# pgvector/pgvector

Measured on AMD Instinct MI355X. Metric: QPS @ recall@10 (IVFFlat, 1M x 1536d), higher is better.
Workload: dtype f32

## Files before the change

### pgvector_amd/csrc/kernels_mfma.hip

```cpp
#include "pgv_device.h"

#include <algorithm>
#include <cfloat>

namespace pgv {

namespace {

typedef float f32x16 __attribute__((ext_vector_type(16)));
typedef _Float16 f16x8 __attribute__((ext_vector_type(8)));
typedef unsigned int u32x4 __attribute__((ext_vector_type(4)));

constexpr int kSliceBytes = 128;
#ifndef PGV_ARGMIN_AUX
#define PGV_ARGMIN_AUX 0
#endif
constexpr int kCand = 4;
constexpr int kWide = 8;

template <typename T> struct MfmaCfg;
template <> struct MfmaCfg<float> {
    static constexpr int WM = 2, WN = 2, TM = 2, TN = 2;
};
template <> struct MfmaCfg<__half> {
// ... 449 lines not shown
__global__ __launch_bounds__(256) void argmin_merge_kernel(int64_t n, int nparts, int lg, const float *__restrict__ part_val,
                                                           const int32_t *__restrict__ part_idx,
                                                           const float *__restrict__ part_x2,
                                                           const float *__restrict__ part_drop, int32_t *__restrict__ out_idx,
                                                           float *__restrict__ out_val, const L2Lists l2) {
    constexpr int W = NC > 1 ? kWide : 1;
    const int G = 1 << lg;
    const int64_t t = (int64_t)blockIdx.x * blockDim.x + threadIdx.x;
    const int64_t r = t >> lg;
    const int p = (int)(t & (G - 1));
    const bool live = r < n && p < nparts;
    unsigned long long list[NC];
#pragma unroll
    for (int c = 0; c < NC; c++) {
        list[c] = ~0ull;
        if (live) {
            const size_t at = ((size_t)r * nparts + p) * NC + c;
            const float v = part_val[at];
            if (v < INFINITY) list[c] = ((unsigned long long)float_to_key(v) << 32) | (unsigned)part_idx[at];
        }
    }
    float sv[W];
    int sid[W];
#pragma unroll
    for (int c = 0; c < W; c++) {
        unsigned long long best = list[0];
        for (int m = 1; m < G; m <<= 1) {
            const unsigned long long o = __shfl_xor(best, m);
            best = o < best ? o : best;
        }
        if (best == ~0ull) {
            sv[c] = INFINITY;
            sid[c] = 0;
        } else {
            sv[c] = key_to_float((unsigned)(best >> 32));
            sid[c] = (int)(unsigned)(best & 0xffffffffu);
        }
        if (list[0] == best && best != ~0ull) {
#pragma unroll
            for (int j = 0; j + 1 < NC; j++) list[j] = list[j + 1];
            list[NC - 1] = ~0ull;
        }
    }
    if constexpr (NC > 1) {
        float dropped = live ? part_drop[(size_t)r * nparts + p] : INFINITY;
        if (list[0] != ~0ull) dropped = fminf(dropped, key_to_float((unsigned)(list[0] >> 32)));
        for (int m = 1; m < G; m <<= 1) dropped = fminf(dropped, __shfl_xor(dropped, m));
        if (r < n && p == 0) finish_l2(r, sv, sid, dropped, part_x2[r], out_idx, l2);
    } else {
        if (r < n && p == 0) finish_ip(r, sv[0], sid[0], out_idx, out_val);
    }
}

template <typename T>
__global__ __launch_bounds__(256) void center_norms_kernel(const char *__restrict__ centers, int k, int nvec,
                                                           float *__restrict__ bias, unsigned *__restrict__ cmax2) {
    const int c = blockIdx.x * 4 + (threadIdx.x >> 6);
    if (c >= k) return;
    const int lane = threadIdx.x & (kWave - 1);
    const char *row = centers + (size_t)c * nvec * sizeof(Raw16);
    float acc = 0.f;
    for (int v = lane; v < nvec; v += kWave) {
        const Raw16 x = load16(row + (size_t)v * sizeof(Raw16));
        acc = accum_slice<T, 1>(acc, x, x);
    }
    for (int m = 32; m > 0; m >>= 1) acc += __shfl_xor(acc, m);
    if (lane == 0) {
        bias[c] = acc;
        atomicMax(cmax2, __float_as_uint(acc));
    }
}

template <typename T>
__global__ __launch_bounds__(256) void recheck_kernel(const char *__restrict__ rows, const char *__restrict__ centers,
                                                      int k, int nvec, const L2Lists l2, int32_t *__restrict__ out_idx,
                                                      int *__restrict__ fb_count,
                                                      int32_t *__restrict__ fb_rows,
                                                      unsigned long long *__restrict__ packed) {
    const int64_t p = (int64_t)blockIdx.x * 4 + (threadIdx.x >> 6);
    if (p >= *l2.u_count) return;
    const int64_t r = l2.u_rows[p];
    const int lane = threadIdx.x & (kWave - 1);
    const size_t row_bytes = (size_t)nvec * sizeof(Raw16);
    const char *row = rows + (size_t)r * row_bytes;
    const float cm2 = __uint_as_float(*l2.cmax2), x2 = l2.u_x2[p];
    const float v0 = l2.u_val[p * kWide];
    int ncheck = 2;
    while (ncheck < kWide && !out_of_band(l2.u_val[p * kWide + ncheck], v0, x2, cm2, l2.gamma, l2.gamma_x)) ncheck++;
    float bv = INFINITY;
    int bid = 0x7fffffff;
    for (int c0 = 0; c0 < ncheck; c0 += kCand) {
        int id[kCand];
        const char *cp[kCand];
#pragma unroll
        for (int c = 0; c < kCand; c++) {
            id[c] = l2.u_cand[p * kWide + (c0 + c < ncheck ? c0 + c : c0)];
            cp[c] = centers + (size_t)id[c] * row_bytes;
        }
        float d[kCand] = {0.f, 0.f, 0.f, 0.f};
        for (int v = lane; v < nvec; v += kWave) {
            const Raw16 x = load16(row + (size_t)v * sizeof(Raw16));
#pragma unroll
            for (int c = 0; c < kCand; c++) d[c] = accum_slice<T, 0>(d[c], x, load16(cp[c] + (size_t)v * sizeof(Raw16)));
        }
        for (int m = 32; m > 0; m >>= 1) {
#pragma unroll
            for (int c = 0; c < kCand; c++) d[c] += __shfl_xor(d[c], m);
        }
#pragma unroll
        for (int c = 0; c < kCand; c++)
            if (c0 + c < ncheck && l2.u_val[p * kWide + c0 + c] < INFINITY &&
                (d[c] < bv || (d[c] == bv && d[c] < INFINITY && id[c] < bid))) {
                bv = d[c];
                bid = id[c];
            }
    }
    if (lane != 0) return;
    out_idx[r] = bid == 0x7fffffff ? 0 : bid;
    if (k > kWide) {
        const bool list_ok = ncheck < kWide;
        if (!(list_ok && out_of_band(l2.u_drop[p], v0, x2, cm2, l2.gamma, l2.gamma_x))) {
            packed[r] = ~0ull;
            fb_rows[atomicAdd(fb_count, 1)] = (int32_t)r;
        }
    }
}

__global__ __launch_bounds__(256) void redo_finish_kernel(const int *__restrict__ fb_count,
                                                          const int32_t *__restrict__ fb_rows,
                                                          const unsigned long long *__restrict__ packed,
                                                          int32_t *__restrict__ out_idx) {
    const int64_t p = (int64_t)blockIdx.x * 256 + threadIdx.x;
    if (p >= *fb_count) return;
    const int64_t r = fb_rows[p];
    const unsigned long long e = packed[r];
    out_idx[r] = e == ~0ull ? 0 : (int32_t)(unsigned)(e & 0xffffffffu);
}

template <typename T>
__global__ __launch_bounds__(256) void chosen_distance_kernel(const char *__restrict__ rows, int64_t n,
                                                              const char *__restrict__ centers, int nvec,
                                                              const int32_t *__restrict__ idx,
                                                              float *__restrict__ out_val) {
    const int64_t r = (int64_t)blockIdx.x * 4 + (threadIdx.x >> 6);
    if (r >= n) return;
    const int lane = threadIdx.x & (kWave - 1);
    const size_t row_bytes = (size_t)nvec * sizeof(Raw16);
    const char *row = rows + (size_t)r * row_bytes;
    const char *cp = centers + (size_t)idx[r] * row_bytes;
    float d0 = 0.f, d1 = 0.f;
    int v = lane;
    for (; v + kWave < nvec; v += 2 * kWave) {
        const Raw16 x0 = load16(row + (size_t)v * sizeof(Raw16)), x1 = load16(row + (size_t)(v + kWave) * sizeof(Raw16));
        const Raw16 c0 = load16(cp + (size_t)v * sizeof(Raw16)), c1 = load16(cp + (size_t)(v + kWave) * sizeof(Raw16));
        d0 = accum_slice<T, 0>(d0, x0, c0);
        d1 = accum_slice<T, 0>(d1, x1, c1);
    }
    if (v < nvec) d0 = accum_slice<T, 0>(d0, load16(row + (size_t)v * sizeof(Raw16)), load16(cp + (size_t)v * sizeof(Raw16)));
    float d = d0 + d1;
    for (int m = 32; m > 0; m >>= 1) d += __shfl_xor(d, m);
    if (lane == 0) out_val[r] = d < INFINITY ? d : FLT_MAX;
}

__global__ void add_count_kernel(const int *u_count, const int *fb_count, double *acc, double rows) {
    acc[0] += (double)*fb_count;
    acc[1] += rows;
    acc[2] += (double)*u_count;
}

template <typename T, int MODE>
int launch_mfma_t(pgv_ctx *ctx, const RowGeom &g, const void *rows, int64_t n, const void *centers, int k,
                  const float *bias, int32_t *out_idx, float *out_val, const L2Lists &l2 = L2Lists()) {
    using C = MfmaCfg<T>;
    constexpr int BM = C::WM * C::TM * 32, BN = C::WN * C::TN * 32;
    constexpr int threads = C::WM * C::WN * 64;
    constexpr int NC = MODE == 0 ? kCand : 1;
    const size_t lds = 2 * (size_t)(BM + BN) * kSliceBytes + sizeof(float) * BM;
    auto kern = mfma_argmin_kernel<T, MODE>;
    PGV_HIP(hipFuncSetAttribute(reinterpret_cast<const void *>(kern), hipFuncAttributeMaxDynamicSharedMemorySize,
                                (int)lds));
    const int64_t row_tiles = (n + BN - 1) / BN;
    static const int env_tiles = [] {
        const char *e = getenv("PGV_ARGMIN_PART_TILES");
        return e ? atoi(e) : -1;
    }();
    const int center_tiles = (k + BM - 1) / BM;
    const bool split = MODE != 0 || sizeof(T) == 2 || row_tiles < 2 * (int64_t)ctx->num_cus;
    const int auto_tiles = row_tiles < 2 * (int64_t)ctx->num_cus ? 1 : (sizeof(T) == 2 ? (MODE == 0 ? 4 : 2) : 1);
    int part_tiles = env_tiles < 0 ? (split ? auto_tiles : center_tiles) : (env_tiles == 0 ? center_tiles : env_tiles);
    int nparts = (center_tiles + part_tiles - 1) / part_tiles;
    if (nparts > 64) {
        part_tiles = (center_tiles + 63) / 64;
        nparts = (center_tiles + part_tiles - 1) / part_tiles;
    }
    float *part_val = nullptr, *part_x2 = nullptr, *part_drop = nullptr;
    int32_t *part_idx = nullptr;
    int64_t grid = row_tiles;
    const bool norms_pass = MODE == 0 && (nparts > 1 || sizeof(T) == 2);
    if (nparts > 1 || norms_pass) {
        const size_t pv = sizeof(float) * (size_t)n * nparts * NC;
        const size_t pd = sizeof(float) * (size_t)n * nparts;
        PGV_TRY(ctx->mf_d.ensure(2 * pv + pd + sizeof(float) * (size_t)n + 64));
        part_val = ctx->mf_d.as<float>();
        part_idx = reinterpret_cast<int32_t *>(ctx->mf_d.as<char>() + pv);
        part_drop = reinterpret_cast<float *>(ctx->mf_d.as<char>() + 2 * pv);
        part_x2 = reinterpret_cast<float *>(ctx->mf_d.as<char>() + 2 * pv + pd);
        if (nparts > 1) grid = 8 * ((row_tiles + 7) / 8) * nparts;
    }
    if (grid > 0x7fffffff) PGV_FAIL(PGV_ERR_ARG, "assignment: too many workgroups");
    if (norms_pass) {
        unsigned *max_bits = reinterpret_cast<unsigned *>(part_x2 + n);
        PGV_HIP(hipMemsetAsync(max_bits, 0, sizeof(unsigned), ctx->stream));
        PGV_TRY(launch_row_norms(ctx, sizeof(T) == 4 ? PGV_F32 : PGV_F16, g, rows, n, part_x2, max_bits));
    }
    hipLaunchKernelGGL(kern, dim3((unsigned)grid), dim3(threads), lds, ctx->stream, static_cast<const char *>(rows), n,
                       static_cast<const char *>(centers), k, g.nvec, bias, static_cast<const char *>(ctx->zeros.p),
                       out_idx, out_val, l2, nparts, part_tiles, part_val, part_idx, part_x2, part_drop);
    PGV_HIP(hipGetLastError());
    if (nparts > 1) {
        int lg = 0;
        while ((1 << lg) < nparts) lg++;
        const int64_t threads_total = n << lg;
        hipLaunchKernelGGL(argmin_merge_kernel<NC>, dim3((unsigned)((threads_total + 255) / 256)), dim3(256), 0, ctx->stream, n,
                           nparts, lg, part_val, part_idx, part_x2, part_drop, out_idx, out_val, l2);
        PGV_HIP(hipGetLastError());
    }
    return PGV_OK;
}

template <typename T>
int launch_mfma_mode(pgv_ctx *ctx, int mode, const RowGeom &g, const void *rows, int64_t n, const void *centers, int k,
                     int32_t *out_idx, float *out_val) {
    if (mode == 1) return launch_mfma_t<T, 1>(ctx, g, rows, n, centers, k, nullptr, out_idx, out_val);
    if (mode == 3) return launch_mfma_t<T, 3>(ctx, g, rows, n, centers, k, nullptr, out_idx, out_val);

    const pgv_dtype dtype = sizeof(T) == 4 ? PGV_F32 : PGV_F16;
    PGV_TRY(ctx->mf_a.ensure(sizeof(float) * (size_t)k + 64));
    PGV_TRY(ctx->mf_b.ensure((sizeof(int32_t) + sizeof(float)) * (size_t)n * kWide + 2 * sizeof(float) * (size_t)n));
    PGV_TRY(ctx->mf_c.ensure((2 * sizeof(int32_t) + sizeof(unsigned long long)) * (size_t)n + 16));
    float *bias = ctx->mf_a.as<float>();
    unsigned *cmax2 = reinterpret_cast<unsigned *>(bias + k);
    int *u_count = reinterpret_cast<int *>(cmax2 + 1);
    int *fb_count = u_count + 1;
    int32_t *u_cand = ctx->mf_b.as<int32_t>();
    float *u_val = reinterpret_cast<float *>(u_cand + (size_t)n * kWide);
    unsigned long long *packed = ctx->mf_c.as<unsigned long long>();
    int32_t *u_rows = reinterpret_cast<int32_t *>(packed + n);
    int32_t *fb_rows = u_rows + n;
    PGV_HIP(hipMemsetAsync(cmax2, 0, 3 * sizeof(int), ctx->stream));
    hipLaunchKernelGGL(center_norms_kernel<T>, dim3((k + 3) / 4), dim3(256), 0, ctx->stream,
                       static_cast<const char *>(centers), k, g.nvec, bias, cmax2);
    L2Lists l2;
    l2.cmax2 = cmax2;
    const ExpansionBound eb = argmin_bound(ctx, g.ld);
    l2.gamma = eb.gamma;
    l2.gamma_x = eb.gamma_exact;
    l2.u_count = u_count;
    l2.u_rows = u_rows;
    l2.u_cand = u_cand;
    l2.u_val = u_val;
    l2.u_drop = u_val + (size_t)n * kWide;
    l2.u_x2 = l2.u_drop + n;
    PGV_TRY((launch_mfma_t<T, 0>(ctx, g, rows, n, centers, k, bias, out_idx, nullptr, l2)));
    hipLaunchKernelGGL(recheck_kernel<T>, dim3((unsigned)((n + 3) / 4)), dim3(256), 0, ctx->stream,
                       static_cast<const char *>(rows), static_cast<const char *>(centers), k, g.nvec, l2, out_idx, fb_count,
                       fb_rows, packed);
    PGV_HIP(hipGetLastError());
    if (k > kWide) {
        PGV_TRY(launch_argmin_listed(ctx, 0, dtype, g, rows, n, centers, k, fb_rows, fb_count, packed));
        hipLaunchKernelGGL(redo_finish_kernel, dim3((unsigned)((n + 255) / 256)), dim3(256), 0, ctx->stream, fb_count,
                           fb_rows, packed, out_idx);
        PGV_HIP(hipGetLastError());
    }
    if (out_val) {
        hipLaunchKernelGGL(chosen_distance_kernel<T>, dim3((unsigned)((n + 3) / 4)), dim3(256), 0, ctx->stream,
                           static_cast<const char *>(rows), n, static_cast<const char *>(centers), g.nvec, out_idx,
                           out_val);
        PGV_HIP(hipGetLastError());
    }
    if (ctx->profiling && ctx->stats_dev.p) {
        hipLaunchKernelGGL(add_count_kernel, dim3(1), dim3(1), 0, ctx->stream, u_count, fb_count,
                           ctx->stats_dev.as<double>() + 2, (double)n);
        PGV_HIP(hipGetLastError());
    }
    return PGV_OK;
}

constexpr int kScanQueries = 32;

constexpr int kScanWaves = 4;

template <typename T, int METRIC, int NW, bool NT, int NQ, int NS = 2, bool SH = false>
__global__ __launch_bounds__(NW * 64) __attribute__((amdgpu_waves_per_eu(NS == 3 ? 2 : 3, NS == 3 ? 2 : 3))) void mfma_scan_kernel(
    const char *__restrict__ rows, const char *__restrict__ queries, const ScanTask *__restrict__ tasks,
    const int *__restrict__ ntasks_ptr, int *__restrict__ task_counter, const ScanPair *__restrict__ pairs,
    const float *__restrict__ row_norms, int nvec, const char *__restrict__ zeros16, float *__restrict__ out,
    const float *__restrict__ qscale) {
    static_assert(!SH || (METRIC == 0 && sizeof(T) == 2), "the shadow scan: fp16 rows, L2");
    constexpr int ROWS = 32 * NW;
    constexpr int NGROUPS = (NQ + ROWS) / 8;
    constexpr int NDMA = (NGROUPS + NW - 1) / NW;
    constexpr int STAGE = (NQ + ROWS) * kSliceBytes;
    static_assert(NS == 2 || (NS == 3 && NQ == 32 && NGROUPS % NW == 0), "three stages: the 32-query form only");
    __shared__ __attribute__((aligned(16))) char smem[NS * STAGE];
    __shared__ int64_t pair_rel[NQ];
    __shared__ float2 pair_ts[SH ? NQ : 1];
    __shared__ int lds_task;
    auto value = [&](float acc, float rn) -> float {
        if constexpr (SH)
            return acc;
        else
            return METRIC == 0 ? fmaf(-2.f, acc, rn) : -acc;
    };
    auto shadow_values = [&](auto &acc, int n, float rn, auto slot) {
#pragma unroll
        for (int r = 0; r < n; r++) {
            const float2 ts = pair_ts[slot(r)];
            acc[r] = fmaf(-ts.y, acc[r], rn + ts.x);
        }
    };

    const int lane = threadIdx.x & (kWave - 1);
    const int wave = __builtin_amdgcn_readfirstlane(threadIdx.x >> 6);
    const int l31 = lane & 31, half = lane >> 5;
    const unsigned sw = (unsigned)(l31 >> 1) & 7u;
    const size_t row_bytes = (size_t)nvec * sizeof(Raw16);
    const int nslices = (nvec + 7) / 8;
    const int ntasks = *ntasks_ptr;
    const unsigned lds0 = (unsigned)(size_t)(__attribute__((address_space(3))) char *)smem;
    const int drow = lane >> 3, dpos = lane & 7;

    if (threadIdx.x == 0) lds_task = atomicAdd(task_counter, 1);
    __syncthreads();
    for (;;) {
        const int t = lds_task;
        if (t >= ntasks) {
            if (threadIdx.x == 0 && atomicAdd(task_counter + 1, 1) == (int)gridDim.x - 1) {
                task_counter[0] = 0;
                task_counter[1] = 0;
            }
            return;
        }
        int next = 0;
        if (threadIdx.x == 0) next = atomicAdd(task_counter, 1);
        const ScanTask task = tasks[t];
        const int np = task.npairs;
        if ((int)threadIdx.x < NQ) {
            const ScanPair pr = pairs[task.pair0 + ((int)threadIdx.x < np ? (int)threadIdx.x : np - 1)];
            pair_rel[threadIdx.x] = pr.out_rel + task.row0;
            if constexpr (SH) {
                pair_ts[threadIdx.x] = make_float2(__int_as_float(pr.pad), qscale[pr.query]);
            }
        }
        const char *src[NDMA];
#pragma unroll
        for (int j = 0; j < NDMA; j++) {
            const int crow = (wave + NW * j) * 8 + drow;
            if (crow < NQ) {
                const ScanPair pr = pairs[task.pair0 + (crow < np ? crow : np - 1)];
                src[j] = queries + (size_t)pr.query * row_bytes;
            } else {
                const int r = crow - NQ;
                src[j] = rows + ((size_t)task.row0 + (size_t)(r < task.nrows ? r : task.nrows - 1)) * row_bytes;
            }
        }
        const bool narrow = np <= 16;
        const bool upper = NQ > 32 && np > 32;
        const bool past_caches = NT && task.pad == 0;
        auto issue_stage = [&](int sl, int buf) {
#pragma unroll
            for (int j = 0; j < NDMA; j++) {
                const int g8 = wave + NW * j;
                if (NGROUPS % NW != 0 && g8 >= NGROUPS) break;
                if (narrow && g8 >= 2 && g8 < NQ / 8) continue;
                if (NQ > 32 && !upper && g8 >= 4 && g8 < NQ / 8) continue;
                const int v = dpos ^ ((4 * (g8 & 1) + (drow >> 1)) & 7);
                const int vi = sl * 8 + v;
                const char *p = vi < nvec ? src[j] + (size_t)vi * sizeof(Raw16) : zeros16;
                char *dst = smem + (size_t)buf * STAGE + (size_t)g8 * 8 * kSliceBytes;
                if (NT && past_caches && g8 >= NQ / 8)
                    __builtin_amdgcn_global_load_lds((const __attribute__((address_space(1))) void *)p,
                                                     (__attribute__((address_space(3))) void *)dst, 16, 0, 2);
                else
                    __builtin_amdgcn_global_load_lds((const __attribute__((address_space(1))) void *)p,
                                                     (__attribute__((address_space(3))) void *)dst, 16, 0, 0);
            }
        };
        const int j32 = wave * 32 + l31;
        if constexpr (NQ > 32) {
          if (!narrow && upper) {
            f32x16 accl, accu, suml, sumu;
#pragma unroll
            for (int r = 0; r < 16; r++) {
                accl[r] = 0.f;
                accu[r] = 0.f;
                suml[r] = 0.f;
                sumu[r] = 0.f;
            }
            const int quarter = (nslices + 3) >> 2;
            int in_quarter = 0;
            const unsigned a_lane = (unsigned)l31 * kSliceBytes;
            const unsigned b_lane = (unsigned)(NQ + wave * 32 + l31) * kSliceBytes;
            issue_stage(0, 0);
            for (int sl = 0; sl < nslices; sl++) {
                __builtin_amdgcn_s_waitcnt(0x0070);
                __builtin_amdgcn_s_barrier();
                if (sl + 1 < nslices) issue_stage(sl + 1, (sl + 1) & 1);
                const unsigned sbase = lds0 + (unsigned)(sl & 1) * STAGE;
                if (upper) {
#pragma unroll
                    for (int c = 0; c < 4; c++) {
                        const unsigned x = (((unsigned)(2 * c + half)) ^ sw) << 4;
                        u32x4 a, au, b;
                        asm volatile("ds_read_b128 %0, %3\n\tds_read_b128 %1, %3 offset:4096\n\tds_read_b128 %2, %4\n\t"
                                     "s_waitcnt lgkmcnt(0)"
                                     : "=&v"(a), "=&v"(au), "=&v"(b)
                                     : "v"(sbase + a_lane + x), "v"(sbase + b_lane + x)
                                     : "memory");
                        Mma<T>::run(accl, a, b);
                        Mma<T>::run(accu, au, b);
                    }
                } else {
#pragma unroll
                    for (int c = 0; c < 4; c++) {
                        const unsigned x = (((unsigned)(2 * c + half)) ^ sw) << 4;
                        u32x4 a, b;
                        asm volatile("ds_read_b128 %0, %2\n\tds_read_b128 %1, %3\n\ts_waitcnt lgkmcnt(0)"
                                     : "=&v"(a), "=&v"(b)
                                     : "v"(sbase + a_lane + x), "v"(sbase + b_lane + x)
                                     : "memory");
                        Mma<T>::run(accl, a, b);
                    }
                }
                if (++in_quarter == quarter) {
                    in_quarter = 0;
                    suml += accl;
                    sumu += accu;
#pragma unroll
                    for (int r = 0; r < 16; r++) {
                        accl[r] = 0.f;
                        accu[r] = 0.f;
                    }
                }
            }
            suml += accl;
            sumu += accu;
            const int j32w = wave * 32 + l31;
            if (j32w < task.nrows) {
                const float rn = METRIC == 0 ? row_norms[task.row0 + j32w] : 0.f;
                if constexpr (SH) {
                    shadow_values(suml, 16, rn, [&](int r) { return (r & 3) + 8 * (r >> 2) + 4 * half; });
                    if (upper) shadow_values(sumu, 16, rn, [&](int r) { return 32 + (r & 3) + 8 * (r >> 2) + 4 * half; });
                }
                {
                    int64_t rel[16];
#pragma unroll
                    for (int r = 0; r < 16; r++) rel[r] = pair_rel[(r & 3) + 8 * (r >> 2) + 4 * half];
#pragma unroll
                    for (int r = 0; r < 16; r++) out[rel[r] + j32w] = value(suml[r], rn);
                }
                if (upper) {
                    int64_t rel[16];
#pragma unroll
                    for (int r = 0; r < 16; r++) rel[r] = pair_rel[32 + (r & 3) + 8 * (r >> 2) + 4 * half];
#pragma unroll
                    for (int r = 0; r < 16; r++) out[rel[r] + j32w] = value(sumu[r], rn);
                }
            }
          }
        }
        if (!narrow && !upper) {
            f32x16 acc4[4];
#pragma unroll
            for (int e = 0; e < 4; e++)
#pragma unroll
                for (int r = 0; r < 16; r++) acc4[e][r] = 0.f;
            const unsigned a_lane = (unsigned)l31 * kSliceBytes;
            const unsigned b_lane = (unsigned)(NQ + wave * 32 + l31) * kSliceBytes;
            issue_stage(0, 0);
            if (NS == 3 && nslices > 1) issue_stage(1, 1);
            int buf = 0;
            for (int sl = 0; sl < nslices; sl++) {
                if (NS == 3 && sl > 0 && sl + 1 < nslices)
                    __builtin_amdgcn_s_waitcnt(0x0075);
                else
                    __builtin_amdgcn_s_waitcnt(0x0070);
                __builtin_amdgcn_s_barrier();
                if (NS == 3) {
                    if (sl + 2 < nslices) issue_stage(sl + 2, buf == 0 ? 2 : buf - 1);
                } else {
                    if (sl + 1 < nslices) issue_stage(sl + 1, (sl + 1) & 1);
                }
                const unsigned sbase = lds0 + (unsigned)(NS == 3 ? buf : (sl & 1)) * STAGE;
                if (NS == 3) buf = buf == 2 ? 0 : buf + 1;
                if (NS == 3) {
                    u32x4 pa[2], pb[2];
                    const unsigned x0 = (((unsigned)half) ^ sw) << 4;
                    asm volatile("ds_read_b128 %0, %2\n\tds_read_b128 %1, %3"
                                 : "=&v"(pa[0]), "=&v"(pb[0])
                                 : "v"(sbase + a_lane + x0), "v"(sbase + b_lane + x0)
                                 : "memory");
#pragma unroll
                    for (int c = 0; c < 4; c++) {
                        if (c + 1 < 4) {
                            const unsigned x = (((unsigned)(2 * (c + 1) + half)) ^ sw) << 4;
                            asm volatile("ds_read_b128 %0, %2\n\tds_read_b128 %1, %3"
                                         : "=&v"(pa[(c + 1) & 1]), "=&v"(pb[(c + 1) & 1])
                                         : "v"(sbase + a_lane + x), "v"(sbase + b_lane + x)
                                         : "memory");
                            asm volatile("s_waitcnt lgkmcnt(2)" : "+v"(pa[c & 1]), "+v"(pb[c & 1])::"memory");
                        } else {
                            asm volatile("s_waitcnt lgkmcnt(0)" : "+v"(pa[c & 1]), "+v"(pb[c & 1])::"memory");
                        }
                        __builtin_amdgcn_sched_barrier(0);
                        Mma4<T>::run(acc4, pa[c & 1], pb[c & 1], c);
                        __builtin_amdgcn_sched_barrier(0);
                    }
                } else {
#pragma unroll
                    for (int c = 0; c < 4; c++) {
                        const unsigned x = (((unsigned)(2 * c + half)) ^ sw) << 4;
                        u32x4 a, b;
                        asm volatile("ds_read_b128 %0, %2\n\tds_read_b128 %1, %3\n\ts_waitcnt lgkmcnt(0)"
                                     : "=&v"(a), "=&v"(b)
                                     : "v"(sbase + a_lane + x), "v"(sbase + b_lane + x)
                                     : "memory");
                        Mma4<T>::run(acc4, a, b, c);
                    }
                }
            }
            f32x16 acc = (acc4[0] + acc4[1]) + (acc4[2] + acc4[3]);
            if constexpr (SH)
                shadow_values(acc, 16, j32 < task.nrows ? row_norms[task.row0 + j32] : 0.f,
                              [&](int r) { return (r & 3) + 8 * (r >> 2) + 4 * half; });
            int64_t rel[16];
#pragma unroll
            for (int r = 0; r < 16; r++) rel[r] = pair_rel[(r & 3) + 8 * (r >> 2) + 4 * half];
            if (j32 < task.nrows) {
                const float rn = METRIC == 0 ? row_norms[task.row0 + j32] : 0.f;
#pragma unroll
                for (int r = 0; r < 16; r++)
                    out[rel[r] + j32] = value(acc[r], rn);
            }
        }
        if (narrow) {
            const int l15 = lane & 15, kg = lane >> 4;
            const unsigned sw15 = (unsigned)(l15 >> 1) & 7u;
            f32x4 c04[4], c14[4];
#pragma unroll
            for (int e = 0; e < 4; e++) {
                c04[e] = f32x4{0.f, 0.f, 0.f, 0.f};
                c14[e] = f32x4{0.f, 0.f, 0.f, 0.f};
            }
            const unsigned a_lane = (unsigned)l15 * kSliceBytes;
            const unsigned b_lane = (unsigned)(NQ + wave * 32 + l15) * kSliceBytes;
            issue_stage(0, 0);
            for (int sl = 0; sl < nslices; sl++) {
                __builtin_amdgcn_s_waitcnt(0x0070);
                __builtin_amdgcn_s_barrier();
                if (sl + 1 < nslices) issue_stage(sl + 1, (sl + 1) & 1);
                const unsigned sbase = lds0 + (unsigned)(sl & 1) * STAGE;
#pragma unroll
                for (int c = 0; c < 2; c++) {
                    const unsigned x = (((unsigned)(kg + 4 * c)) ^ sw15) << 4;
                    u32x4 a, b0, b1;
                    asm volatile("ds_read_b128 %0, %3\n\tds_read_b128 %1, %4\n\tds_read_b128 %2, %4 offset:2048\n\t"
                                 "s_waitcnt lgkmcnt(0)"
                                 : "=&v"(a), "=&v"(b0), "=&v"(b1)
                                 : "v"(sbase + a_lane + x), "v"(sbase + b_lane + x)
                                 : "memory");
                    if (sl & 1)
                        Mma16x4<T>::run(c04, c14, a, b0, b1, c + 2);
                    else
                        Mma16x4<T>::run(c04, c14, a, b0, b1, c);
                }
            }
            f32x4 c0 = (c04[0] + c04[1]) + (c04[2] + c04[3]), c1 = (c14[0] + c14[1]) + (c14[2] + c14[3]);
            int64_t rel[4];
#pragma unroll
            for (int r = 0; r < 4; r++) rel[r] = pair_rel[4 * kg + r];
            const int ja = wave * 32 + l15, jb = ja + 16;
            const float rna = (METRIC == 0 && ja < task.nrows) ? row_norms[task.row0 + ja] : 0.f;
            const float rnb = (METRIC == 0 && jb < task.nrows) ? row_norms[task.row0 + jb] : 0.f;
            if constexpr (SH) {
                shadow_values(c0, 4, rna, [&](int r) { return 4 * kg + r; });
                shadow_values(c1, 4, rnb, [&](int r) { return 4 * kg + r; });
            }
            if (ja < task.nrows) {
#pragma unroll
                for (int r = 0; r < 4; r++) out[rel[r] + ja] = value(c0[r], rna);
            }
            if (jb < task.nrows) {
#pragma unroll
                for (int r = 0; r < 4; r++) out[rel[r] + jb] = value(c1[r], rnb);
            }
        }
        __builtin_amdgcn_s_waitcnt(0xc07f);
        __builtin_amdgcn_s_barrier();
        if (threadIdx.x == 0) lds_task = next;
        __syncthreads();
    }
}

template <typename T>
__global__ __launch_bounds__(256) void row_norms_kernel(const char *__restrict__ rows, int64_t n, int nvec,
                                                        float *__restrict__ out, unsigned *__restrict__ max_bits) {
    const int64_t r = (int64_t)blockIdx.x * 4 + (threadIdx.x >> 6);
    if (r >= n) return;
    const int lane = threadIdx.x & (kWave - 1);
    const char *row = rows + (size_t)r * nvec * sizeof(Raw16);
    float acc = 0.f;
    for (int v = lane; v < nvec; v += kWave) {
        const Raw16 x = load16(row + (size_t)v * sizeof(Raw16));
        acc = accum_slice<T, 1>(acc, x, x);
    }
    for (int m = 32; m > 0; m >>= 1) acc += __shfl_xor(acc, m);
    if (lane == 0) {
        out[r] = acc;
        if (max_bits && __float_as_uint(acc) > __hip_atomic_load(max_bits, __ATOMIC_RELAXED, __HIP_MEMORY_SCOPE_AGENT))
            atomicMax(max_bits, __float_as_uint(acc));
    }
}

}

bool mfma_argmin_supported(int mode, int64_t n, int k) { return (mode == 0 || mode == 1 || mode == 3) && k >= 64 && n >= 256; }

int launch_argmin_mfma(pgv_ctx *ctx, int mode, pgv_dtype dtype, const RowGeom &g, const void *rows, int64_t n,
                       const void *centers, int k, int32_t *out_idx, float *out_val) {
    if (n <= 0) return PGV_OK;
    if (!ctx->zeros.p) {
        PGV_TRY(ctx->zeros.ensure(256));
        PGV_HIP(hipMemsetAsync(ctx->zeros.p, 0, 256, ctx->stream));
    }
    if (dtype == PGV_F32) return launch_mfma_mode<float>(ctx, mode, g, rows, n, centers, k, out_idx, out_val);
    return launch_mfma_mode<__half>(ctx, mode, g, rows, n, centers, k, out_idx, out_val);
}

}

namespace pgv {

int mfma_scan_rows_per_task() { return 32 * kScanWaves; }
int mfma_scan_queries_per_task() { return kScanQueries; }
int shadow_chain_length(const RowGeom &g16) {
    const int nslices = (g16.nvec + 7) / 8;
    const int a = 16 * nslices, b = 32 * ((nslices + 1) / 2), c = 64 * ((nslices + 3) / 4);
    return std::max(a, std::max(b, c));
}
int scan_chain_length(const RowGeom &g, pgv_dtype dtype, bool wide) {
    const int nslices = (g.nvec + 7) / 8, quarter = (nslices + 3) / 4;
    if (dtype == PGV_F32) return std::max(g.ld / 4, wide ? 32 * quarter : 0);
    return std::max(16 * nslices, std::max(32 * ((nslices + 1) / 2), wide ? 64 * quarter : 0));
}
int mfma_scan_queries_per_task_wide() { return 2 * kScanQueries; }

int launch_row_norms(pgv_ctx *ctx, pgv_dtype dtype, const RowGeom &g, const void *rows, int64_t n, float *out,
                     unsigned *max_bits) {
    if (n <= 0) return PGV_OK;
    const dim3 grid((unsigned)((n + 3) / 4));
    if (dtype == PGV_F32)
        hipLaunchKernelGGL(row_norms_kernel<float>, grid, dim3(256), 0, ctx->stream, static_cast<const char *>(rows), n,
                           g.nvec, out, max_bits);
    else
        hipLaunchKernelGGL(row_norms_kernel<__half>, grid, dim3(256), 0, ctx->stream, static_cast<const char *>(rows), n,
                           g.nvec, out, max_bits);
    PGV_HIP(hipGetLastError());
    return PGV_OK;
}

int launch_mfma_scan(pgv_ctx *ctx, pgv_metric metric, pgv_dtype dtype, const RowGeom &g, const void *rows,
                     const void *queries, const ScanTask *tasks, const int *ntasks_dev, int ntasks_bound,
                     const ScanPair *pairs, const float *row_norms, const float *query_norms, float *out,
                     bool stream_rows, int queries_per_task, const float *shadow_scale) {
    if (ntasks_bound <= 0) return PGV_OK;
    if (queries_per_task != 32 && queries_per_task != 64) PGV_FAIL(PGV_ERR_ARG, "mfma scan: %d queries per task", queries_per_task);
    if (metric != PGV_L2SQ && metric != PGV_NEG_IP) PGV_FAIL(PGV_ERR_ARG, "mfma scan: L2 / inner product only");
    if (!ctx->zeros.p) {
        PGV_TRY(ctx->zeros.ensure(256));
        PGV_HIP(hipMemsetAsync(ctx->zeros.p, 0, 256, ctx->stream));
    }
    PGV_TRY(ctx->counters.ensure(256));
    if (!ctx->counters_clean) {
        PGV_HIP(hipMemsetAsync(ctx->counters.p, 0, 256, ctx->stream));
        ctx->counters_clean = true;
    }
    int *counter = ctx->counters.as<int>() + 8;
    int grid = ctx->num_cus * 3;
    if (grid > ntasks_bound) grid = ntasks_bound;
    static const int deep_env = [] {
        const char *e = getenv("PGV_SCAN_DEEP");
        return e ? atoi(e) : -1;
    }();
    const bool deep = queries_per_task == 32 && deep_env != 0 && ntasks_bound <= 2 * ctx->num_cus;
#define PGV_MSCAN_QS(T, M, NT, Q, S, SH)                                                                                  \
    hipLaunchKernelGGL((mfma_scan_kernel<T, M, kScanWaves, NT, Q, S, SH>), dim3(grid), dim3(kScanWaves * 64), 0,          \
                       ctx->stream, static_cast<const char *>(rows), static_cast<const char *>(queries), tasks, ntasks_dev, \
                       counter, pairs, row_norms, g.nvec, static_cast<const char *>(ctx->zeros.p), out, shadow_scale)
#define PGV_MSCAN_Q(T, M, NT, Q, S) PGV_MSCAN_QS(T, M, NT, Q, S, false)
#define PGV_MSCAN_NT(T, M, NT)                   \
    do {                                         \
        if (queries_per_task == 64)              \
            PGV_MSCAN_Q(T, M, NT, 64, 2);         \
        else if (deep)                           \
            PGV_MSCAN_Q(T, M, NT, 32, 3);         \
        else                                     \
            PGV_MSCAN_Q(T, M, NT, 32, 2);         \
    } while (0)
#define PGV_MSCAN(T, M)              \
    do {                             \
        if (stream_rows)             \
            PGV_MSCAN_NT(T, M, true); \
        else                         \
            PGV_MSCAN_NT(T, M, false); \
    } while (0)
    if (shadow_scale) {
        if (metric != PGV_L2SQ || dtype != PGV_F16) PGV_FAIL(PGV_ERR_ARG, "mfma scan: the shadow form is fp16 L2 only");
#define PGV_MSCAN_SH(NT)                                   \
    do {                                                   \
        if (queries_per_task == 64)                        \
            PGV_MSCAN_QS(__half, 0, NT, 64, 2, true);       \
        else if (deep)                                     \
            PGV_MSCAN_QS(__half, 0, NT, 32, 3, true);       \
        else                                               \
            PGV_MSCAN_QS(__half, 0, NT, 32, 2, true);       \
    } while (0)
        if (stream_rows)
            PGV_MSCAN_SH(true);
        else
            PGV_MSCAN_SH(false);
#undef PGV_MSCAN_SH
    } else if (dtype == PGV_F32) {
        if (metric == PGV_L2SQ)
            PGV_MSCAN(float, 0);
        else
            PGV_MSCAN(float, 1);
    } else {
        if (metric == PGV_L2SQ)
            PGV_MSCAN(__half, 0);
        else
            PGV_MSCAN(__half, 1);
    }
#undef PGV_MSCAN
#undef PGV_MSCAN_NT
#undef PGV_MSCAN_Q
#undef PGV_MSCAN_QS
    PGV_HIP(hipGetLastError());
    return PGV_OK;
}

}
```

Measured before the change: 1.407 million.

## Double-buffer task index and claim next task during slice loop

Task claiming moves from the end of each task to right after the first stage load is issued. The claimed index is published into a second LDS slot after the first in-loop barrier, so the tail __syncthreads is removed. Row-norm loads are also hoisted ahead of the main loop so their latency overlaps the MFMA work. This takes the atomic round trip and one block barrier off the critical path between tasks, at the cost of keeping row norms in registers through the loop and relying on barrier ordering for the parity slot.

```diff
diff --git a/pgvector_amd/csrc/kernels_mfma.hip b/pgvector_amd/csrc/kernels_mfma.hip
--- a/pgvector_amd/csrc/kernels_mfma.hip
+++ b/pgvector_amd/csrc/kernels_mfma.hip
@@ -778,7 +778,7 @@
     __shared__ __attribute__((aligned(16))) char smem[NS * STAGE];
     __shared__ int64_t pair_rel[NQ];
     __shared__ float2 pair_ts[SH ? NQ : 1];
-    __shared__ int lds_task;
+    __shared__ int lds_task[2];
     auto value = [&](float acc, float rn) -> float {
         if constexpr (SH)
             return acc;
@@ -803,10 +803,10 @@
     const unsigned lds0 = (unsigned)(size_t)(__attribute__((address_space(3))) char *)smem;
     const int drow = lane >> 3, dpos = lane & 7;
 
-    if (threadIdx.x == 0) lds_task = atomicAdd(task_counter, 1);
+    if (threadIdx.x == 0) lds_task[0] = atomicAdd(task_counter, 1);
     __syncthreads();
-    for (;;) {
-        const int t = lds_task;
+    for (int par = 0;; par ^= 1) {
+        const int t = lds_task[par];
         if (t >= ntasks) {
             if (threadIdx.x == 0 && atomicAdd(task_counter + 1, 1) == (int)gridDim.x - 1) {
                 task_counter[0] = 0;
@@ -815,7 +815,16 @@
             return;
         }
         int next = 0;
-        if (threadIdx.x == 0) next = atomicAdd(task_counter, 1);
+        auto claim_next = [&] {
+            if (threadIdx.x == 0) {
+                auto *counter = (__attribute__((address_space(1))) int *)task_counter;
+                asm volatile("" : "+v"(counter));
+                next = __hip_atomic_fetch_add(counter, 1, __ATOMIC_RELAXED, __HIP_MEMORY_SCOPE_AGENT);
+            }
+        };
+        auto publish_next = [&] {
+            if (threadIdx.x == 0) lds_task[par ^ 1] = next;
+        };
         const ScanTask task = tasks[t];
         const int np = task.npairs;
         if ((int)threadIdx.x < NQ) {
@@ -875,9 +884,11 @@
             const unsigned a_lane = (unsigned)l31 * kSliceBytes;
             const unsigned b_lane = (unsigned)(NQ + wave * 32 + l31) * kSliceBytes;
             issue_stage(0, 0);
+            claim_next();
             for (int sl = 0; sl < nslices; sl++) {
                 __builtin_amdgcn_s_waitcnt(0x0070);
                 __builtin_amdgcn_s_barrier();
+                if (sl == 0) publish_next();
                 if (sl + 1 < nslices) issue_stage(sl + 1, (sl + 1) & 1);
                 const unsigned sbase = lds0 + (unsigned)(sl & 1) * STAGE;
                 if (upper) {
@@ -952,6 +963,9 @@
             const unsigned b_lane = (unsigned)(NQ + wave * 32 + l31) * kSliceBytes;
             issue_stage(0, 0);
             if (NS == 3 && nslices > 1) issue_stage(1, 1);
+            claim_next();
+            float rn = 0.f;
+            if (NQ == 32 && METRIC == 0 && j32 < task.nrows) rn = row_norms[task.row0 + j32];
             int buf = 0;
             for (int sl = 0; sl < nslices; sl++) {
                 if (NS == 3 && sl > 0 && sl + 1 < nslices)
@@ -959,6 +973,7 @@
                 else
                     __builtin_amdgcn_s_waitcnt(0x0070);
                 __builtin_amdgcn_s_barrier();
+                if (sl == 0) publish_next();
                 if (NS == 3) {
                     if (sl + 2 < nslices) issue_stage(sl + 2, buf == 0 ? 2 : buf - 1);
                 } else {
@@ -1003,14 +1018,13 @@
                 }
             }
             f32x16 acc = (acc4[0] + acc4[1]) + (acc4[2] + acc4[3]);
+            if (NQ > 32 && METRIC == 0 && j32 < task.nrows) rn = row_norms[task.row0 + j32];
             if constexpr (SH)
-                shadow_values(acc, 16, j32 < task.nrows ? row_norms[task.row0 + j32] : 0.f,
-                              [&](int r) { return (r & 3) + 8 * (r >> 2) + 4 * half; });
+                shadow_values(acc, 16, rn, [&](int r) { return (r & 3) + 8 * (r >> 2) + 4 * half; });
             int64_t rel[16];
 #pragma unroll
             for (int r = 0; r < 16; r++) rel[r] = pair_rel[(r & 3) + 8 * (r >> 2) + 4 * half];
             if (j32 < task.nrows) {
-                const float rn = METRIC == 0 ? row_norms[task.row0 + j32] : 0.f;
 #pragma unroll
                 for (int r = 0; r < 16; r++)
                     out[rel[r] + j32] = value(acc[r], rn);
@@ -1028,9 +1042,14 @@
             const unsigned a_lane = (unsigned)l15 * kSliceBytes;
             const unsigned b_lane = (unsigned)(NQ + wave * 32 + l15) * kSliceBytes;
             issue_stage(0, 0);
+            claim_next();
+            const int ja = wave * 32 + l15, jb = ja + 16;
+            const float rna = (METRIC == 0 && ja < task.nrows) ? row_norms[task.row0 + ja] : 0.f;
+            const float rnb = (METRIC == 0 && jb < task.nrows) ? row_norms[task.row0 + jb] : 0.f;
             for (int sl = 0; sl < nslices; sl++) {
                 __builtin_amdgcn_s_waitcnt(0x0070);
                 __builtin_amdgcn_s_barrier();
+                if (sl == 0) publish_next();
                 if (sl + 1 < nslices) issue_stage(sl + 1, (sl + 1) & 1);
                 const unsigned sbase = lds0 + (unsigned)(sl & 1) * STAGE;
 #pragma unroll
@@ -1052,9 +1071,6 @@
             int64_t rel[4];
 #pragma unroll
             for (int r = 0; r < 4; r++) rel[r] = pair_rel[4 * kg + r];
-            const int ja = wave * 32 + l15, jb = ja + 16;
-            const float rna = (METRIC == 0 && ja < task.nrows) ? row_norms[task.row0 + ja] : 0.f;
-            const float rnb = (METRIC == 0 && jb < task.nrows) ? row_norms[task.row0 + jb] : 0.f;
             if constexpr (SH) {
                 shadow_values(c0, 4, rna, [&](int r) { return 4 * kg + r; });
                 shadow_values(c1, 4, rnb, [&](int r) { return 4 * kg + r; });
@@ -1070,8 +1086,6 @@
         }
         __builtin_amdgcn_s_waitcnt(0xc07f);
         __builtin_amdgcn_s_barrier();
-        if (threadIdx.x == 0) lds_task = next;
-        __syncthreads();
     }
 }
 
```

Result: no change. 1.433 million (median of 6 runs) (+1.9%).

## Prefetch next scan task header, pair table and row norms into LDS during slice loop

Applied to the files above, without the earlier changes.

For the two-stage scan kernel, the next task's header, its pair table and (for the shadow form) the query scales are fetched by asynchronous global-to-LDS loads. These fetches are spread across the first slice iterations of the current task, so the serial global reads between tasks are taken off the critical path. Row norms for the current tile are also DMA'd into LDS at loop start instead of being read from global in the epilogue. The cost is more LDS use, double-buffered pair tables, and tricky ordering of waits and barriers that could break correctness if any step is mis-synchronised.

```diff
diff --git a/pgvector_amd/csrc/kernels_mfma.hip b/pgvector_amd/csrc/kernels_mfma.hip
--- a/pgvector_amd/csrc/kernels_mfma.hip
+++ b/pgvector_amd/csrc/kernels_mfma.hip
@@ -775,10 +775,27 @@
     constexpr int NDMA = (NGROUPS + NW - 1) / NW;
     constexpr int STAGE = (NQ + ROWS) * kSliceBytes;
     static_assert(NS == 2 || (NS == 3 && NQ == 32 && NGROUPS % NW == 0), "three stages: the 32-query form only");
+    constexpr bool PF = NS == 2;
+    constexpr int NQJ = NQ / (8 * NW);
+    constexpr int kHeaderSteps = SH ? 6 : 5;
+    static_assert(NQ % (8 * NW) == 0 && NQ <= kWave, "query rows: whole DMA groups; one wavefront fetches a pair table");
     __shared__ __attribute__((aligned(16))) char smem[NS * STAGE];
-    __shared__ int64_t pair_rel[NQ];
-    __shared__ float2 pair_ts[SH ? NQ : 1];
+    __shared__ int64_t pair_rel[PF ? 1 : NQ];
+    __shared__ float2 pair_ts[!PF && SH ? NQ : 1];
+    __shared__ __attribute__((aligned(16))) ScanPair pair_raw[PF ? 2 : 1][PF ? kWave : 1];
+    __shared__ float pair_qs[PF && SH ? 2 : 1][PF && SH ? kWave : 1];
+    __shared__ __attribute__((aligned(8))) int lds_hdr[kWave];
+    __shared__ float lds_rn[PF && METRIC == 0 ? ROWS : 1];
     __shared__ int lds_task;
+    __shared__ int lds_next;
+    int cur = 0;
+    int64_t cur_row0 = 0;
+    auto rel_of = [&](int slot) -> int64_t {
+        if constexpr (PF)
+            return pair_raw[cur][slot].out_rel + cur_row0;
+        else
+            return pair_rel[slot];
+    };
     auto value = [&](float acc, float rn) -> float {
         if constexpr (SH)
             return acc;
@@ -788,7 +805,11 @@
     auto shadow_values = [&](auto &acc, int n, float rn, auto slot) {
 #pragma unroll
         for (int r = 0; r < n; r++) {
-            const float2 ts = pair_ts[slot(r)];
+            float2 ts;
+            if constexpr (PF)
+                ts = make_float2(__int_as_float(pair_raw[cur][slot(r)].pad), pair_qs[cur][slot(r)]);
+            else
+                ts = pair_ts[slot(r)];
             acc[r] = fmaf(-ts.y, acc[r], rn + ts.x);
         }
     };
@@ -803,8 +824,61 @@
     const unsigned lds0 = (unsigned)(size_t)(__attribute__((address_space(3))) char *)smem;
     const int drow = lane >> 3, dpos = lane & 7;
 
-    if (threadIdx.x == 0) lds_task = atomicAdd(task_counter, 1);
+    int next = 0;
+    bool have = false;
+    auto dma4 = [&](const void *g, void *l) {
+        __builtin_amdgcn_global_load_lds((const __attribute__((address_space(1))) void *)g,
+                                         (__attribute__((address_space(3))) void *)l, 4, 0, 0);
+    };
+    auto header_step = [&](int s, bool now) {
+        if (s == 0) {
+            int off = 0;
+            asm volatile("" : "+v"(off));
+            if (threadIdx.x == 0) next = atomicAdd(task_counter + off, 1);
+            return;
+        }
+        if (s == 1) {
+            if (threadIdx.x == 0) lds_next = next;
+            return;
+        }
+        if (wave != 0) return;
+        if (now) __builtin_amdgcn_s_waitcnt(0x0070);
+        const int nxt = cur ^ 1;
+        int lane = (int)threadIdx.x;
+        asm volatile("" : "+v"(lane));
+        if (s == 2) {
+            const int nx = lds_next;
+            have = __builtin_amdgcn_readfirstlane(nx) < ntasks;
+            if (have) dma4(reinterpret_cast<const int *>(tasks + nx) + (lane < 5 ? lane : 5), lds_hdr);
+        } else if (s == 3) {
+            if (have) {
+                const int pair0 = lds_hdr[3], np = lds_hdr[4];
+                __builtin_amdgcn_global_load_lds(
+                    (const __attribute__((address_space(1))) void *)(pairs + (pair0 + (lane < np ? lane : np - 1))),
+                    (__attribute__((address_space(3))) void *)pair_raw[nxt], 16, 0, 0);
+            }
+        } else if (s == 4) {
+            if constexpr (SH) {
+                if (have) dma4(qscale + pair_raw[nxt][lane].query, pair_qs[nxt]);
+            }
+        }
+    };
+    auto slice_link = [&](int sl) {
+        asm volatile("" : "+s"(sl));
+        if (sl < kHeaderSteps - 1) header_step(sl, false);
+    };
+    const int hstep = nslices < kHeaderSteps ? nslices : kHeaderSteps;
+
+    if (threadIdx.x == 0) {
+        const int first = atomicAdd(task_counter, 1);
+        lds_task = first;
+        if constexpr (PF) lds_next = first;
+    }
     __syncthreads();
+    if constexpr (PF) {
+        for (int s = 2; s < kHeaderSteps; s++) header_step(s, true);
+        __syncthreads();
+    }
     for (;;) {
         const int t = lds_task;
         if (t >= ntasks) {
@@ -814,29 +888,53 @@
             }
             return;
         }
-        int next = 0;
-        if (threadIdx.x == 0) next = atomicAdd(task_counter, 1);
-        const ScanTask task = tasks[t];
+        int next3 = 0;
+        if constexpr (!PF) {
+            if (threadIdx.x == 0) next3 = atomicAdd(task_counter, 1);
+        }
+        ScanTask task;
+        const char *src[NDMA];
+        if constexpr (PF) {
+            cur ^= 1;
+            task.row0 = (int64_t)(((uint64_t)(unsigned)__builtin_amdgcn_readfirstlane(lds_hdr[1]) << 32) |
+                                  (uint64_t)(unsigned)__builtin_amdgcn_readfirstlane(lds_hdr[0]));
+            task.nrows = __builtin_amdgcn_readfirstlane(lds_hdr[2]);
+            task.pair0 = __builtin_amdgcn_readfirstlane(lds_hdr[3]);
+            task.npairs = __builtin_amdgcn_readfirstlane(lds_hdr[4]);
+            task.pad = __builtin_amdgcn_readfirstlane(lds_hdr[5]);
+            cur_row0 = task.row0;
+#pragma unroll
+            for (int j = 0; j < NDMA; j++) {
+                const int crow = (wave + NW * j) * 8 + drow;
+                if (j < NQJ) {
+                    src[j] = queries + (size_t)pair_raw[cur][crow].query * row_bytes;
+                } else {
+                    const int r = crow - NQ;
+                    src[j] = rows + ((size_t)task.row0 + (size_t)(r < task.nrows ? r : task.nrows - 1)) * row_bytes;
+                }
+            }
+        } else {
+            task = tasks[t];
+            if ((int)threadIdx.x < NQ) {
+                const ScanPair pr = pairs[task.pair0 + ((int)threadIdx.x < task.npairs ? (int)threadIdx.x : task.npairs - 1)];
+                pair_rel[threadIdx.x] = pr.out_rel + task.row0;
+                if constexpr (SH) {
+                    pair_ts[threadIdx.x] = make_float2(__int_as_float(pr.pad), qscale[pr.query]);
+                }
+            }
+#pragma unroll
+            for (int j = 0; j < NDMA; j++) {
+                const int crow = (wave + NW * j) * 8 + drow;
+                if (crow < NQ) {
+                    const ScanPair pr = pairs[task.pair0 + (crow < task.npairs ? crow : task.npairs - 1)];
+                    src[j] = queries + (size_t)pr.query * row_bytes;
+                } else {
+                    const int r = crow - NQ;
+                    src[j] = rows + ((size_t)task.row0 + (size_t)(r < task.nrows ? r : task.nrows - 1)) * row_bytes;
+                }
+            }
+        }
         const int np = task.npairs;
-        if ((int)threadIdx.x < NQ) {
-            const ScanPair pr = pairs[task.pair0 + ((int)threadIdx.x < np ? (int)threadIdx.x : np - 1)];
-            pair_rel[threadIdx.x] = pr.out_rel + task.row0;
-            if constexpr (SH) {
-                pair_ts[threadIdx.x] = make_float2(__int_as_float(pr.pad), qscale[pr.query]);
-            }
-        }
-        const char *src[NDMA];
-#pragma unroll
-        for (int j = 0; j < NDMA; j++) {
-            const int crow = (wave + NW * j) * 8 + drow;
-            if (crow < NQ) {
-                const ScanPair pr = pairs[task.pair0 + (crow < np ? crow : np - 1)];
-                src[j] = queries + (size_t)pr.query * row_bytes;
-            } else {
-                const int r = crow - NQ;
-                src[j] = rows + ((size_t)task.row0 + (size_t)(r < task.nrows ? r : task.nrows - 1)) * row_bytes;
-            }
-        }
         const bool narrow = np <= 16;
         const bool upper = NQ > 32 && np > 32;
         const bool past_caches = NT && task.pad == 0;
@@ -860,6 +958,14 @@
             }
         };
         const int j32 = wave * 32 + l31;
+        auto load_norms = [&]() {
+            if constexpr (PF && METRIC == 0) {
+                if (wave < 2) {
+                    const int i = wave * 64 + lane;
+                    dma4(row_norms + task.row0 + (i < task.nrows ? i : task.nrows - 1), lds_rn + wave * 64);
+                }
+            }
+        };
         if constexpr (NQ > 32) {
           if (!narrow && upper) {
             f32x16 accl, accu, suml, sumu;
@@ -875,9 +981,11 @@
             const unsigned a_lane = (unsigned)l31 * kSliceBytes;
             const unsigned b_lane = (unsigned)(NQ + wave * 32 + l31) * kSliceBytes;
             issue_stage(0, 0);
+            load_norms();
             for (int sl = 0; sl < nslices; sl++) {
                 __builtin_amdgcn_s_waitcnt(0x0070);
                 __builtin_amdgcn_s_barrier();
+                if constexpr (PF) slice_link(sl);
                 if (sl + 1 < nslices) issue_stage(sl + 1, (sl + 1) & 1);
                 const unsigned sbase = lds0 + (unsigned)(sl & 1) * STAGE;
                 if (upper) {
@@ -920,7 +1028,7 @@
             sumu += accu;
             const int j32w = wave * 32 + l31;
             if (j32w < task.nrows) {
-                const float rn = METRIC == 0 ? row_norms[task.row0 + j32w] : 0.f;
+                const float rn = METRIC == 0 ? lds_rn[j32w] : 0.f;
                 if constexpr (SH) {
                     shadow_values(suml, 16, rn, [&](int r) { return (r & 3) + 8 * (r >> 2) + 4 * half; });
                     if (upper) shadow_values(sumu, 16, rn, [&](int r) { return 32 + (r & 3) + 8 * (r >> 2) + 4 * half; });
@@ -928,14 +1036,14 @@
                 {
                     int64_t rel[16];
 #pragma unroll
-                    for (int r = 0; r < 16; r++) rel[r] = pair_rel[(r & 3) + 8 * (r >> 2) + 4 * half];
+                    for (int r = 0; r < 16; r++) rel[r] = rel_of((r & 3) + 8 * (r >> 2) + 4 * half);
 #pragma unroll
                     for (int r = 0; r < 16; r++) out[rel[r] + j32w] = value(suml[r], rn);
                 }
                 if (upper) {
                     int64_t rel[16];
 #pragma unroll
-                    for (int r = 0; r < 16; r++) rel[r] = pair_rel[32 + (r & 3) + 8 * (r >> 2) + 4 * half];
+                    for (int r = 0; r < 16; r++) rel[r] = rel_of(32 + (r & 3) + 8 * (r >> 2) + 4 * half);
 #pragma unroll
                     for (int r = 0; r < 16; r++) out[rel[r] + j32w] = value(sumu[r], rn);
                 }
@@ -952,6 +1060,7 @@
             const unsigned b_lane = (unsigned)(NQ + wave * 32 + l31) * kSliceBytes;
             issue_stage(0, 0);
             if (NS == 3 && nslices > 1) issue_stage(1, 1);
+            load_norms();
             int buf = 0;
             for (int sl = 0; sl < nslices; sl++) {
                 if (NS == 3 && sl > 0 && sl + 1 < nslices)
@@ -959,6 +1068,7 @@
                 else
                     __builtin_amdgcn_s_waitcnt(0x0070);
                 __builtin_amdgcn_s_barrier();
+                if constexpr (PF) slice_link(sl);
                 if (NS == 3) {
                     if (sl + 2 < nslices) issue_stage(sl + 2, buf == 0 ? 2 : buf - 1);
                 } else {
@@ -1004,13 +1114,13 @@
             }
             f32x16 acc = (acc4[0] + acc4[1]) + (acc4[2] + acc4[3]);
             if constexpr (SH)
-                shadow_values(acc, 16, j32 < task.nrows ? row_norms[task.row0 + j32] : 0.f,
+                shadow_values(acc, 16, PF ? lds_rn[PF && METRIC == 0 ? j32 : 0] : j32 < task.nrows ? row_norms[task.row0 + j32] : 0.f,
                               [&](int r) { return (r & 3) + 8 * (r >> 2) + 4 * half; });
             int64_t rel[16];
 #pragma unroll
-            for (int r = 0; r < 16; r++) rel[r] = pair_rel[(r & 3) + 8 * (r >> 2) + 4 * half];
+            for (int r = 0; r < 16; r++) rel[r] = rel_of((r & 3) + 8 * (r >> 2) + 4 * half);
             if (j32 < task.nrows) {
-                const float rn = METRIC == 0 ? row_norms[task.row0 + j32] : 0.f;
+                const float rn = PF ? (METRIC == 0 ? lds_rn[PF && METRIC == 0 ? j32 : 0] : 0.f) : METRIC == 0 ? row_norms[task.row0 + j32] : 0.f;
 #pragma unroll
                 for (int r = 0; r < 16; r++)
                     out[rel[r] + j32] = value(acc[r], rn);
@@ -1028,9 +1138,11 @@
             const unsigned a_lane = (unsigned)l15 * kSliceBytes;
             const unsigned b_lane = (unsigned)(NQ + wave * 32 + l15) * kSliceBytes;
             issue_stage(0, 0);
+            load_norms();
             for (int sl = 0; sl < nslices; sl++) {
                 __builtin_amdgcn_s_waitcnt(0x0070);
                 __builtin_amdgcn_s_barrier();
+                if constexpr (PF) slice_link(sl);
                 if (sl + 1 < nslices) issue_stage(sl + 1, (sl + 1) & 1);
                 const unsigned sbase = lds0 + (unsigned)(sl & 1) * STAGE;
 #pragma unroll
@@ -1051,10 +1163,10 @@
             f32x4 c0 = (c04[0] + c04[1]) + (c04[2] + c04[3]), c1 = (c14[0] + c14[1]) + (c14[2] + c14[3]);
             int64_t rel[4];
 #pragma unroll
-            for (int r = 0; r < 4; r++) rel[r] = pair_rel[4 * kg + r];
+            for (int r = 0; r < 4; r++) rel[r] = rel_of(4 * kg + r);
             const int ja = wave * 32 + l15, jb = ja + 16;
-            const float rna = (METRIC == 0 && ja < task.nrows) ? row_norms[task.row0 + ja] : 0.f;
-            const float rnb = (METRIC == 0 && jb < task.nrows) ? row_norms[task.row0 + jb] : 0.f;
+            const float rna = PF ? (METRIC == 0 ? lds_rn[PF && METRIC == 0 ? ja : 0] : 0.f) : (METRIC == 0 && ja < task.nrows) ? row_norms[task.row0 + ja] : 0.f;
+            const float rnb = PF ? (METRIC == 0 ? lds_rn[PF && METRIC == 0 ? jb : 0] : 0.f) : (METRIC == 0 && jb < task.nrows) ? row_norms[task.row0 + jb] : 0.f;
             if constexpr (SH) {
                 shadow_values(c0, 4, rna, [&](int r) { return 4 * kg + r; });
                 shadow_values(c1, 4, rnb, [&](int r) { return 4 * kg + r; });
@@ -1070,8 +1182,15 @@
         }
         __builtin_amdgcn_s_waitcnt(0xc07f);
         __builtin_amdgcn_s_barrier();
-        if (threadIdx.x == 0) lds_task = next;
-        __syncthreads();
+        if constexpr (PF) {
+            for (int s = hstep; s < kHeaderSteps; s++) header_step(s, true);
+            if (threadIdx.x == 0) lds_task = lds_next;
+            __builtin_amdgcn_s_waitcnt(0xc07f);
+            __builtin_amdgcn_s_barrier();
+        } else {
+            if (threadIdx.x == 0) lds_task = next3;
+            __syncthreads();
+        }
     }
 }
 
```

After: 1.414 million before, 1.441 million after, median of 6. About the same (+1.9%).
